# torchkge-team/torchkge

Measured on AMD Instinct MI355X. Metric: link-prediction triples scored/sec (filtered LP eval, both sides), higher is better.
Workload: dtype f32 (f16 hi/lo-split MFMA prefilter + exact f32 recheck; ranks bit-identical to f32)

## Files before the change

### torchkge_amd/csrc/lp_split_recheck.hip

```cpp
#include "lp_split_common.h"
#include "lp_pair_exact.h"

namespace {


__device__ __forceinline__ float recheck_e_segment(const float *__restrict__ T, int64_t ldt, int K, int ci,
                                                   const float *__restrict__ qrow, float *es, float acc)
{
    const int lane = threadIdx.x & 63;
    int k0 = 0;
    if (K >= KGE_PS_KC) {
        float4 e0, e1, e2, e3, e4, e5, e6, e7;
#define KGE_RR_FETCH(IT, KK)                                                                                  \
    {                                                                                                         \
        const int idx_ = lane + 64 * IT, rr_ = idx_ >> 3, pc_ = idx_ & 7;                                     \
        const int rc_ = __shfl(ci, rr_, 64);                                                                  \
        e##IT = *reinterpret_cast<const float4 *>(T + (int64_t)rc_ * ldt + (KK) + pc_ * 4);                   \
    }
#define KGE_RR_STORE(IT)                                                                                      \
    {                                                                                                         \
        const int idx_ = lane + 64 * IT, rr_ = idx_ >> 3, pc_ = idx_ & 7;                                     \
        *reinterpret_cast<float4 *>(es + rr_ * KGE_PS_LD + pc_ * 4) = e##IT;                                  \
    }
#define KGE_RR_ALL(M, ...) M(0, ##__VA_ARGS__) M(1, ##__VA_ARGS__) M(2, ##__VA_ARGS__) M(3, ##__VA_ARGS__) \
                           M(4, ##__VA_ARGS__) M(5, ##__VA_ARGS__) M(6, ##__VA_ARGS__) M(7, ##__VA_ARGS__)
        KGE_RR_ALL(KGE_RR_FETCH, 0)
        for (; k0 + KGE_PS_KC <= K; k0 += KGE_PS_KC) {
            KGE_RR_ALL(KGE_RR_STORE)
            if (k0 + 2 * KGE_PS_KC <= K) { KGE_RR_ALL(KGE_RR_FETCH, k0 + KGE_PS_KC) }
            __builtin_amdgcn_fence(__ATOMIC_SEQ_CST, "wavefront");
            acc = lp_chain_dot(qrow + k0, es + lane * KGE_PS_LD, KGE_PS_KC, acc);
            __builtin_amdgcn_fence(__ATOMIC_SEQ_CST, "wavefront");
        }
#undef KGE_RR_ALL
#undef KGE_RR_STORE
#undef KGE_RR_FETCH
    }
    for (; k0 < K; k0 += KGE_PS_KC) {
        const int kc = min(KGE_PS_KC, K - k0);
        const int pieces = kc >> 2;
        for (int idx = lane; idx < 64 * pieces; idx += 64) {
            const int rr = idx / pieces, pc = idx - rr * pieces;
            const int rc = __shfl(ci, rr, 64);
            *reinterpret_cast<float4 *>(es + rr * KGE_PS_LD + pc * 4) =
                *reinterpret_cast<const float4 *>(T + (int64_t)rc * ldt + k0 + pc * 4);
        }
        __builtin_amdgcn_fence(__ATOMIC_SEQ_CST, "wavefront");
        acc = lp_chain_dot(qrow + k0, es + lane * KGE_PS_LD, kc, acc);
        __builtin_amdgcn_fence(__ATOMIC_SEQ_CST, "wavefront");
    }
    return acc;
}

constexpr int RR_G = 4;

template <int NWV>
__global__ __launch_bounds__(64 * NWV) void split_recheck_regions_kernel(const kge_lp_desc d, const float *__restrict__ s_true,
                                                                        const int32_t *__restrict__ list, int32_t region_cap,
                                                                        const int32_t *__restrict__ region_count, int n_regions,
                                                                        int ldq, int seg_cols, int32_t *raw_count, float *list_stat,
                                                                        int32_t *list_count)
{
    extern __shared__ __attribute__((aligned(16))) float rr_smem[];
    const int tid = threadIdx.x, lane = tid & 63, wv = tid >> 6;
    float *qrows = rr_smem;
    float *es = rr_smem + RR_ROWS * ldq + wv * 64 * KGE_PS_LD;
    const int K = d.K0 + d.K1;
    int n_block = 0;
    auto stage = [&](int64_t q0, int c0, int c1) {
        const int np = (c1 - c0) >> 2;
        for (int idx = tid; idx < RR_ROWS * np; idx += 64 * NWV) {
            const int rr = idx / np, pc = idx - rr * np;
            const int64_t q = min(q0 + rr, d.B - 1);
            const int col = c0 + pc * 4;
            const float4 v = col < d.K0 ? *reinterpret_cast<const float4 *>(d.A0 + q * d.lda0 + col)
                                        : *reinterpret_cast<const float4 *>(d.A1 + q * d.lda1 + (col - d.K0));
            *reinterpret_cast<float4 *>(qrows + rr * ldq + pc * 4) = v;
        }
    };
    auto chain = [&](float acc, int ci, const float *qrow, int c0, int c1) -> float {
        if (c0 < d.K0) acc = recheck_e_segment(d.T0 + c0, d.ldt0, min(c1, d.K0) - c0, ci, qrow, es, acc);
        if (c1 > d.K0 && d.K1 > 0) {
            const int s0 = max(c0, d.K0);
            acc = recheck_e_segment(d.T1 + (s0 - d.K0), d.ldt1, c1 - s0, ci, qrow + (s0 - c0), es, acc);
        }
        return acc;
    };
    for (int reg = blockIdx.x; reg < n_regions; reg += gridDim.x) {
        const int n = (int)min((unsigned)region_count[reg], (unsigned)region_cap);
        if (n == 0) continue;
        n_block += n;
        const int64_t q0 = (int64_t)(reg / 3) * RR_PANEL + (reg % 3) * RR_ROWS;
        const int2 *ent = reinterpret_cast<const int2 *>(list) + (int64_t)reg * region_cap;
        if (K <= seg_cols) {
            __syncthreads();
            stage(q0, 0, K);
            __syncthreads();
            for (int c0 = wv * 64; c0 < n; c0 += NWV * 64) {
                const int pi = c0 + lane;
                const bool valid = pi < n;
                const int2 e = ent[valid ? pi : c0];
                const int qi = e.x, ci = e.y;
                const float acc = chain(0.0f, ci, qrows + (int)(qi - q0) * ldq, 0, K);
                const float sc = lp_epilogue_any(d, acc, qi, ci);
                if (valid && !(sc >= s_true[qi])) atomicSub(&raw_count[qi], 1);
            }
            continue;
        }
        for (int b0 = 0; b0 < n; b0 += NWV * 64 * RR_G) {
            float acc[RR_G];
            int qi[RR_G], ci[RR_G];
#pragma unroll
            for (int g = 0; g < RR_G; ++g) {
                const int c0 = b0 + (g * NWV + wv) * 64;
                const int pi = c0 + lane;
                const int2 e = ent[min(pi < n ? pi : c0, n - 1)];
                qi[g] = e.x; ci[g] = e.y; acc[g] = 0.0f;
            }
            for (int c0 = 0; c0 < K; c0 += seg_cols) {
                const int c1 = min(K, c0 + seg_cols);
                __syncthreads();
                stage(q0, c0, c1);
                __syncthreads();
#pragma unroll
                for (int g = 0; g < RR_G; ++g)
                    if (b0 + (g * NWV + wv) * 64 < n)
                        acc[g] = chain(acc[g], ci[g], qrows + (int)(qi[g] - q0) * ldq, c0, c1);
            }
#pragma unroll
            for (int g = 0; g < RR_G; ++g) {
                const int pi = b0 + (g * NWV + wv) * 64 + lane;
                if (pi < n) {
                    const float sc = lp_epilogue_any(d, acc[g], qi[g], ci[g]);
                    if (!(sc >= s_true[qi[g]])) atomicSub(&raw_count[qi[g]], 1);
                }
            }
        }
    }
    if (tid == 0 && n_block > 0) {
        if (list_stat) atomicAdd(list_stat, (float)n_block);
        if (list_count) atomicAdd(list_count, n_block);
    }
}

}

extern "C" int kge_lp_split_recheck(const kge_lp_desc *d, const float *s_true, const int32_t *list, int32_t cap,
                                    const int32_t *list_count, int32_t *raw_count, float *list_stat, kge_stream_t stream)
{
    int rc = kge_lp_desc_check(d);
    if (rc) return rc;
    if (d->B == 0 || d->N == 0) return 0;
    if (!s_true || !list || cap <= 0 || !list_count || !raw_count) return KGE_EINVAL;
    if (!KGE_LP_IS_MFMA(d->mode)) return KGE_EINVAL;
    const int grid = split_num_cus() * kge_env_int("KGE_SPLIT_RECHECK_WAVES", 160 * 1024 / (2 * 64 * KGE_PS_LD * 4));
    return lp_pair_dispatch<PAIR_STAGED>(*d, [&](auto v) {
        using V = decltype(v);
        if constexpr (V::chain != PAIR_DOT) return KGE_EINVAL;
        else {
            hipLaunchKernelGGL(lp_list_recheck_kernel<V>, dim3(grid), dim3(64), 0, kge_s(stream), *d, s_true, list, cap,
                               list_count, raw_count, list_stat);
            KGE_CHECK_LAUNCH();
            return 0;
        }
    });
}

extern "C" int kge_lp_split_regions(int64_t B)
{
    return (int)(kge_lp_split_rows_padded(B, 1) / RR_PANEL) * 3;
}

static int region_seg_cols(int K)
{
    const int max_ld = kge_env_int("KGE_REGION_MAX_BYTES", 36 * 1024) / (RR_ROWS * 4);
    const int ld_full = K + (((K >> 2) & 1) ? 0 : 4);
    if (ld_full <= max_ld) return K;
    const int seg_ld = min(max_ld, kge_env_int("KGE_REGION_SEG_BYTES", 20 * 1024) / (RR_ROWS * 4));
    int seg = ((seg_ld - 4) / 32) * 32;
    return seg < 32 ? 32 : seg;
}

extern "C" int kge_lp_split_regions_supported(const kge_lp_desc *d)
{
    if (kge_lp_desc_check(d) || !KGE_LP_IS_MFMA(d->mode) || !kge_lp_vec4(*d)) return 0;
    const int K = d->K0 + d->K1;
    if ((K + 2 + 15) / 16 > 32) return 0;
    if (region_seg_cols(K) < K && kge_env_int("KGE_REGION_SEGMENTS", 1) == 0) return 0;
    return 1;
}

extern "C" int kge_lp_split_recheck_regions(const kge_lp_desc *d, const float *s_true, const int32_t *list, int32_t cap,
                                            const int32_t *region_count, int32_t *raw_count, float *list_stat,
                                            int32_t *list_count, kge_stream_t stream)
{
    int rc = kge_lp_desc_check(d);
    if (rc) return rc;
    if (d->B == 0 || d->N == 0) return 0;
    if (!s_true || !list || cap <= 0 || !region_count || !raw_count) return KGE_EINVAL;
    if (!kge_lp_split_regions_supported(d)) return KGE_EINVAL;
    const int n_regions = kge_lp_split_regions(d->B);
    const int32_t region_cap = cap / n_regions;
    if (region_cap <= 0) return KGE_EINVAL;
    const int K = d->K0 + d->K1;
    const int seg = region_seg_cols(K);
    const int ldq = seg + (((seg >> 2) & 1) ? 0 : 4);
    const int nwv = kge_env_int("KGE_RECHECK_REGION_WAVES", 2);
    const int smem = (RR_ROWS * ldq + (nwv == 4 ? 4 : 2) * 64 * KGE_PS_LD) * 4;
    const int want = split_num_cus() * 6;
    const int grid = n_regions < want ? n_regions : want;
    static int attr2[16], attr4[16];
    if (nwv == 4) {
        auto k = split_recheck_regions_kernel<4>;
        if (int e = kge_ensure_dyn_smem(reinterpret_cast<const void *>(k), smem, attr4)) return e;
        hipLaunchKernelGGL(k, dim3(grid), dim3(256), smem, kge_s(stream), *d, s_true, list, region_cap, region_count, n_regions,
                           ldq, seg, raw_count, list_stat, list_count);
    } else {
        auto k = split_recheck_regions_kernel<2>;
        if (int e = kge_ensure_dyn_smem(reinterpret_cast<const void *>(k), smem, attr2)) return e;
        hipLaunchKernelGGL(k, dim3(grid), dim3(128), smem, kge_s(stream), *d, s_true, list, region_cap, region_count, n_regions,
                           ldq, seg, raw_count, list_stat, list_count);
    }
    KGE_CHECK_LAUNCH();
    return 0;
}
```

Before: 1321 billion.

## Split region recheck into region×batch work items with per-operand staging and occupancy-based grid

The recheck kernel now distributes work as (region, batch) items across blocks and uses a lane-parallel ballot to skip empty items, replacing the old one-block-per-region loop. This is meant to fix load imbalance when a few regions hold many candidates. Staging now runs separately for each operand (A0/T0, then A1/T1), which drops the per-element K0 branch. Segment width is chosen per operand, with a smaller default segment for small K. The grid is sized from a cached occupancy query rather than a fixed 6 blocks per CU, at the cost of re-staging the query rows once per batch instead of once per region.

Result: slower. 1251 billion (-5.3%).

```diff
diff --git a/torchkge_amd/csrc/lp_split_recheck.hip b/torchkge_amd/csrc/lp_split_recheck.hip
--- a/torchkge_amd/csrc/lp_split_recheck.hip
+++ b/torchkge_amd/csrc/lp_split_recheck.hip
@@ -58,56 +58,40 @@
 __global__ __launch_bounds__(64 * NWV) void split_recheck_regions_kernel(const kge_lp_desc d, const float *__restrict__ s_true,
                                                                         const int32_t *__restrict__ list, int32_t region_cap,
                                                                         const int32_t *__restrict__ region_count, int n_regions,
-                                                                        int ldq, int seg_cols, int32_t *raw_count, float *list_stat,
-                                                                        int32_t *list_count)
+                                                                        int n_batches, int ldq, int seg_cols, int32_t *raw_count,
+                                                                        float *list_stat, int32_t *list_count)
 {
     extern __shared__ __attribute__((aligned(16))) float rr_smem[];
+    constexpr int BATCH = NWV * 64 * RR_G;
     const int tid = threadIdx.x, lane = tid & 63, wv = tid >> 6;
     float *qrows = rr_smem;
     float *es = rr_smem + RR_ROWS * ldq + wv * 64 * KGE_PS_LD;
-    const int K = d.K0 + d.K1;
     int n_block = 0;
-    auto stage = [&](int64_t q0, int c0, int c1) {
+    auto stage = [&](const float *__restrict__ A, int64_t lda, int64_t q0, int c0, int c1) {
         const int np = (c1 - c0) >> 2;
         for (int idx = tid; idx < RR_ROWS * np; idx += 64 * NWV) {
             const int rr = idx / np, pc = idx - rr * np;
             const int64_t q = min(q0 + rr, d.B - 1);
-            const int col = c0 + pc * 4;
-            const float4 v = col < d.K0 ? *reinterpret_cast<const float4 *>(d.A0 + q * d.lda0 + col)
-                                        : *reinterpret_cast<const float4 *>(d.A1 + q * d.lda1 + (col - d.K0));
-            *reinterpret_cast<float4 *>(qrows + rr * ldq + pc * 4) = v;
+            *reinterpret_cast<float4 *>(qrows + rr * ldq + pc * 4) =
+                *reinterpret_cast<const float4 *>(A + q * lda + c0 + pc * 4);
         }
     };
-    auto chain = [&](float acc, int ci, const float *qrow, int c0, int c1) -> float {
-        if (c0 < d.K0) acc = recheck_e_segment(d.T0 + c0, d.ldt0, min(c1, d.K0) - c0, ci, qrow, es, acc);
-        if (c1 > d.K0 && d.K1 > 0) {
-            const int s0 = max(c0, d.K0);
-            acc = recheck_e_segment(d.T1 + (s0 - d.K0), d.ldt1, c1 - s0, ci, qrow + (s0 - c0), es, acc);
-        }
-        return acc;
-    };
-    for (int reg = blockIdx.x; reg < n_regions; reg += gridDim.x) {
-        const int n = (int)min((unsigned)region_count[reg], (unsigned)region_cap);
-        if (n == 0) continue;
-        n_block += n;
-        const int64_t q0 = (int64_t)(reg / 3) * RR_PANEL + (reg % 3) * RR_ROWS;
-        const int2 *ent = reinterpret_cast<const int2 *>(list) + (int64_t)reg * region_cap;
-        if (K <= seg_cols) {
-            __syncthreads();
-            stage(q0, 0, K);
-            __syncthreads();
-            for (int c0 = wv * 64; c0 < n; c0 += NWV * 64) {
-                const int pi = c0 + lane;
-                const bool valid = pi < n;
-                const int2 e = ent[valid ? pi : c0];
-                const int qi = e.x, ci = e.y;
-                const float acc = chain(0.0f, ci, qrows + (int)(qi - q0) * ldq, 0, K);
-                const float sc = lp_epilogue_any(d, acc, qi, ci);
-                if (valid && !(sc >= s_true[qi])) atomicSub(&raw_count[qi], 1);
-            }
-            continue;
-        }
-        for (int b0 = 0; b0 < n; b0 += NWV * 64 * RR_G) {
+    const int64_t n_items = (int64_t)n_regions * n_batches;
+    for (int64_t base = blockIdx.x; base < n_items; base += (int64_t)64 * gridDim.x) {
+        const int64_t it_l = base + (int64_t)lane * gridDim.x;
+        int n_l = 0;
+        if (it_l < n_items) {
+            n_l = (int)min((unsigned)region_count[it_l % n_regions], (unsigned)region_cap);
+            if ((it_l / n_regions) * BATCH >= n_l) n_l = 0;
+        }
+        for (uint64_t todo = __ballot(n_l > 0); todo; todo &= todo - 1) {
+            const int l = __builtin_ctzll(todo);
+            const int64_t item = base + (int64_t)l * gridDim.x;
+            const int n = __shfl(n_l, l, 64);
+            const int reg = (int)(item % n_regions), b0 = (int)(item / n_regions) * BATCH;
+            if (b0 == 0) n_block += n;
+            const int64_t q0 = (int64_t)(reg / 3) * RR_PANEL + (reg % 3) * RR_ROWS;
+            const int2 *ent = reinterpret_cast<const int2 *>(list) + (int64_t)reg * region_cap;
             float acc[RR_G];
             int qi[RR_G], ci[RR_G];
 #pragma unroll
@@ -117,15 +101,20 @@
                 const int2 e = ent[min(pi < n ? pi : c0, n - 1)];
                 qi[g] = e.x; ci[g] = e.y; acc[g] = 0.0f;
             }
-            for (int c0 = 0; c0 < K; c0 += seg_cols) {
-                const int c1 = min(K, c0 + seg_cols);
-                __syncthreads();
-                stage(q0, c0, c1);
-                __syncthreads();
+            for (int op = 0; op < 2; ++op) {
+                const int Kop = op ? d.K1 : d.K0;
+                const float *A = op ? d.A1 : d.A0, *T = op ? d.T1 : d.T0;
+                const int64_t lda = op ? d.lda1 : d.lda0, ldt = op ? d.ldt1 : d.ldt0;
+                for (int c0 = 0; c0 < Kop; c0 += seg_cols) {
+                    const int c1 = min(Kop, c0 + seg_cols);
+                    __syncthreads();
+                    stage(A, lda, q0, c0, c1);
+                    __syncthreads();
 #pragma unroll
-                for (int g = 0; g < RR_G; ++g)
-                    if (b0 + (g * NWV + wv) * 64 < n)
-                        acc[g] = chain(acc[g], ci[g], qrows + (int)(qi[g] - q0) * ldq, c0, c1);
+                    for (int g = 0; g < RR_G; ++g)
+                        if (b0 + (g * NWV + wv) * 64 < n)
+                            acc[g] = recheck_e_segment(T + c0, ldt, c1 - c0, ci[g], qrows + (int)(qi[g] - q0) * ldq, es, acc[g]);
+                }
             }
 #pragma unroll
             for (int g = 0; g < RR_G; ++g) {
@@ -171,13 +160,13 @@
     return (int)(kge_lp_split_rows_padded(B, 1) / RR_PANEL) * 3;
 }
 
-static int region_seg_cols(int K)
+static int region_seg_cols(int K, int Kop)
 {
     const int max_ld = kge_env_int("KGE_REGION_MAX_BYTES", 36 * 1024) / (RR_ROWS * 4);
-    const int ld_full = K + (((K >> 2) & 1) ? 0 : 4);
-    if (ld_full <= max_ld) return K;
-    const int seg_ld = min(max_ld, kge_env_int("KGE_REGION_SEG_BYTES", 20 * 1024) / (RR_ROWS * 4));
-    int seg = ((seg_ld - 4) / 32) * 32;
+    const int seg_ld = min(max_ld, kge_env_int("KGE_REGION_SEG_BYTES", (K > 256 ? 20 : 9) * 1024) / (RR_ROWS * 4));
+    const int ld_full = Kop + (((Kop >> 2) & 1) ? 0 : 4);
+    if (ld_full <= seg_ld) return Kop;
+    const int seg = ((seg_ld - 4) / 32) * 32;
     return seg < 32 ? 32 : seg;
 }
 
@@ -185,9 +174,7 @@
 {
     if (kge_lp_desc_check(d) || !KGE_LP_IS_MFMA(d->mode) || !kge_lp_vec4(*d)) return 0;
     const int K = d->K0 + d->K1;
-    if ((K + 2 + 15) / 16 > 32) return 0;
-    if (region_seg_cols(K) < K && kge_env_int("KGE_REGION_SEGMENTS", 1) == 0) return 0;
-    return 1;
+    return (K + 2 + 15) / 16 <= 32;
 }
 
 extern "C" int kge_lp_split_recheck_regions(const kge_lp_desc *d, const float *s_true, const int32_t *list, int32_t cap,
@@ -202,25 +189,33 @@
     const int n_regions = kge_lp_split_regions(d->B);
     const int32_t region_cap = cap / n_regions;
     if (region_cap <= 0) return KGE_EINVAL;
-    const int K = d->K0 + d->K1;
-    const int seg = region_seg_cols(K);
+    const int seg = region_seg_cols(d->K0 + d->K1, d->K0 > d->K1 ? d->K0 : d->K1);
     const int ldq = seg + (((seg >> 2) & 1) ? 0 : 4);
-    const int nwv = kge_env_int("KGE_RECHECK_REGION_WAVES", 2);
-    const int smem = (RR_ROWS * ldq + (nwv == 4 ? 4 : 2) * 64 * KGE_PS_LD) * 4;
-    const int want = split_num_cus() * 6;
-    const int grid = n_regions < want ? n_regions : want;
-    static int attr2[16], attr4[16];
-    if (nwv == 4) {
-        auto k = split_recheck_regions_kernel<4>;
-        if (int e = kge_ensure_dyn_smem(reinterpret_cast<const void *>(k), smem, attr4)) return e;
-        hipLaunchKernelGGL(k, dim3(grid), dim3(256), smem, kge_s(stream), *d, s_true, list, region_cap, region_count, n_regions,
-                           ldq, seg, raw_count, list_stat, list_count);
-    } else {
-        auto k = split_recheck_regions_kernel<2>;
-        if (int e = kge_ensure_dyn_smem(reinterpret_cast<const void *>(k), smem, attr2)) return e;
-        hipLaunchKernelGGL(k, dim3(grid), dim3(128), smem, kge_s(stream), *d, s_true, list, region_cap, region_count, n_regions,
-                           ldq, seg, raw_count, list_stat, list_count);
-    }
+    const int nwv = kge_env_int("KGE_RECHECK_REGION_WAVES", 2) == 4 ? 4 : 2;
+    const int smem = (RR_ROWS * ldq + nwv * 64 * KGE_PS_LD) * 4;
+    const int batch = nwv * 64 * RR_G;
+    const int n_batches = (region_cap + batch - 1) / batch;
+    const int64_t n_items = (int64_t)n_regions * n_batches;
+    auto launch = [&](auto k, int *attr, int (*slots)[2]) -> int {
+        if (int e = kge_ensure_dyn_smem(reinterpret_cast<const void *>(k), smem, attr)) return e;
+        int dev = 0;
+        if (hipGetDevice(&dev) != hipSuccess || dev < 0 || dev >= 16) return KGE_EINVAL;
+        if (slots[dev][0] != smem) {
+            int nb = 0;
+            if (hipOccupancyMaxActiveBlocksPerMultiprocessor(&nb, k, 64 * nwv, smem) != hipSuccess || nb <= 0) return KGE_EINVAL;
+            slots[dev][1] = nb;
+            slots[dev][0] = smem;
+        }
+        const int per_cu = slots[dev][1];
+        const int64_t want = (int64_t)split_num_cus() * (per_cu + (per_cu + 1) / 2);
+        const int grid = (int)(n_items < want ? n_items : want);
+        hipLaunchKernelGGL(k, dim3(grid), dim3(64 * nwv), smem, kge_s(stream), *d, s_true, list, region_cap, region_count,
+                           n_regions, n_batches, ldq, seg, raw_count, list_stat, list_count);
+        return 0;
+    };
+    static int attr2[16], attr4[16], slots2[16][2], slots4[16][2];
+    if (int e = nwv == 4 ? launch(split_recheck_regions_kernel<4>, attr4, slots4)
+                         : launch(split_recheck_regions_kernel<2>, attr2, slots2)) return e;
     KGE_CHECK_LAUNCH();
     return 0;
 }
```
